# IlzeAmandaA/VAE-GP-ODE

Hardware: AMD Instinct MI355X
Metric: latent_trajectories_per_sec (higher is better)
Workload: dtype f32; 1 GPU; configs[1]: ode1 DF q=6 M=100 S=256 T=16 batch=256; step = full ELBO training step (encoder, GP draw, rk4 rollout, decoder, ELBO, backward, Adam), L=1; global_batch=256, mc_draws=1, solver=rk4 (3/8 rule), parallelism=dp1, hip_graph=True, graph_scope=whole, gp_side_stream=True, batchnorm=per-process statistics

## Files before the change

### include/gpode.h

```cpp
#ifndef GPODE_H
#define GPODE_H
#include <stddef.h>
#ifdef __cplusplus
extern "C" {
#endif

#define GPODE_KERNEL_RBF 0
#define GPODE_KERNEL_DF 1
#define GPODE_METHOD_EULER 0
#define GPODE_METHOD_RK4 1
#define GPODE_METHOD_MIDPOINT 2
#define GPODE_METHOD_DOPRI5 3

const char* gpode_version(void);
const char* gpode_last_error(void);
const char* gpode_last_launch(void);
int gpode_supported(int kernel, int Di, int Do);

int gpode_cache_sizes(int kernel, int Di, int Do, int M, int S, size_t* pack_floats, size_t* ws_floats);

int gpode_cache_build_fwd(int kernel, int Di, int Do, int M, int S,
                          const float* raw_ell, const float* raw_var, const float* Z,
                          const float* Um, const float* Us_packed,
                          const float* eps_u, const float* rff_w, const float* rff_eps, const float* rff_u,
// ... 170 lines not shown
                 int relu, float* scratch, void* stream);
int gpode_bn_stats(const float* x, const float* gamma, const float* beta, float* save_mean, float* save_invstd, float* running_mean,
                   float* running_var, long long* num_batches_tracked, float momentum, float eps, float* table, int B, int C, int HW,
                   float* scratch, void* stream);
int gpode_bn_moments(const float* x, float* moments, int B, int C, int HW, float* scratch, void* stream);
int gpode_bn_finalize(const float* gathered, int nranks, const float* gamma, const float* beta, float* save_mean, float* save_invstd,
                      float* running_mean, float* running_var, long long* num_batches_tracked, float momentum, float eps, float* table,
                      int C, void* stream);
int gpode_bn_apply(const float* x, const float* table, float* y, int B, int C, int HW, int relu, void* stream);
int gpode_bn_bwd_sums(const float* x, const float* gy, const float* gamma, const float* beta, const float* save_mean,
                      const float* save_invstd, float* sums, int B, int C, int HW, int relu, float* scratch, void* stream);
int gpode_bn_bwd_apply(const float* x, const float* gy, const float* gamma, const float* beta, const float* save_mean,
                       const float* save_invstd, const float* sums_gathered, const float* weights, int nranks, float count_all,
                       float* gx, float* ggamma, float* gbeta, float* gx_chansum, int B, int C, int HW, int relu, float* scratch,
                       void* stream);
void gpode_defer_reductions(int mode);
int gpode_flush_reductions(void* stream);
int gpode_dec10_bn_wgrad_scratch_floats(void);
int gpode_dec10_bn_bwd_sums_wgrad(const float* c, const float* gy, const float* w, const float* gamma, const float* beta, const float* save_mean,
                                  const float* save_invstd, float* sums, float* gw, float* gbias, int B, float* scratch, float* wscratch,
                                  void* stream);
int gpode_dec10_bn_scratch_floats(void);
int gpode_dec10_bn_bwd_sums(const float* c, const float* gy, const float* w, const float* gamma, const float* beta, const float* save_mean,
                            const float* save_invstd, float* sums, int B, float* scratch, void* stream);
int gpode_dec10_bn_bwd_apply(const float* c, const float* gy, const float* w, const float* gamma, const float* beta, const float* save_mean,
                             const float* save_invstd, const float* sums_gathered, const float* weights, int nranks, float count_all,
                             float* gc, float* ggamma, float* gbeta, float* gc_chansum, int B, float* scratch, void* stream);
int gpode_bn_eval(const float* x, const float* gy, const float* gamma, const float* beta, const float* running_mean,
                  const float* running_var, float eps, float* out, int B, int C, int HW, int relu, void* stream);
int gpode_bn_eval_table(const float* gamma, const float* beta, const float* running_mean, const float* running_var, float eps, float* table,
// ... 109 lines not shown
```

### vae-gp-ode_amd/_lib.py

```python
import ctypes
import os

_HERE = os.path.dirname(os.path.abspath(__file__))
LIB_PATH = os.path.join(_HERE, 'libgpode_hip.so')

_vp = ctypes.c_void_p
_i = ctypes.c_int
_f = ctypes.c_float
_sz = ctypes.c_size_t
_sz_p = ctypes.POINTER(_sz)

SIGNATURES = {
    'gpode_version': (ctypes.c_char_p, []),
    'gpode_last_error': (ctypes.c_char_p, []),
    'gpode_last_launch': (ctypes.c_char_p, []),
    'gpode_supported': (_i, [_i, _i, _i]),
    'gpode_cache_sizes': (_i, [_i, _i, _i, _i, _i, _sz_p, _sz_p]),
    'gpode_cache_build_fwd': (_i, [_i] * 5 + [_vp] * 20),
    'gpode_cache_bwd_sizes': (_i, [_i, _i, _i, _i, _i, _sz_p]),
    'gpode_cache_build_bwd': (_i, [_i] * 5 + [_vp] * 13 + [_i, _vp]),
    'gpode_cache_bwd_prepare': (_i, [_i] * 5 + [_vp] * 2 + [_vp]),
    'gpode_cache_info': (_i, [_vp, ctypes.POINTER(_i), _vp]),
    'gpode_cache_pivots': (_i, [_vp, ctypes.POINTER(_f), _vp]),
    'gpode_set_backward_solves': (_i, [_i]),
# ... 41 lines not shown
    'gpode_kern_cache': (_i, [_i] * 4 + [_vp] * 8 + [_vp]),
    'gpode_compute_nu_ws': (_i, [_i] * 4 + [_sz_p]),
    'gpode_compute_nu': (_i, [_i] * 4 + [_vp] * 5 + [_vp]),
    'gpode_f_update': (_i, [_i] * 4 + [_vp] * 5 + [_i, _vp, _vp, _vp]),
    'gpode_conv2d_fwd': (_i, [_vp] * 4 + [_i] * 10 + [_vp]),
    'gpode_conv2d_bwd_data': (_i, [_vp] * 4 + [_i] * 10 + [_vp]),
    'gpode_conv2d_fwd_bs': (_i, [_vp, _sz] + [_vp] * 3 + [_i] * 10 + [_vp]),
    'gpode_conv2d_bwd_weight_bs': (_i, [_vp, _sz] + [_vp] * 4 + [_i] * 10 + [_vp]),
    'gpode_convT_fwd_stats_scratch': (_sz, [_i]),
    'gpode_convT_fwd_stats': (_i, [_vp] * 5 + [_i] * 10 + [_vp] * 6 + [_vp, _f, _f, _vp, _vp, _i, _vp]),
    'gpode_conv_wgrad_scratch': (_sz, [_i, _i, _i, _i]),
    'gpode_conv2d_bwd_weight': (_i, [_vp] * 5 + [_i] * 10 + [_vp]),
    'gpode_bn_scratch': (_sz, [_i, _i]),
    'gpode_bn_fwd': (_i, [_vp] * 8 + [_vp, _f, _f, _i, _i, _i, _i, _vp, _vp]),
    'gpode_bn_bwd': (_i, [_vp] * 10 + [_i, _i, _i, _i, _vp, _vp]),
    'gpode_conv2d_bwd_data_bn': (_i, [_vp] * 5 + [_i] * 10 + [_vp]),
    'gpode_conv2d_bwd_weight_bn': (_i, [_vp] * 6 + [_i] * 10 + [_vp]),
    'gpode_bn_stats': (_i, [_vp] * 7 + [_vp, _f, _f, _vp, _i, _i, _i, _vp, _vp]),
    'gpode_bn_moments': (_i, [_vp, _vp, _i, _i, _i, _vp, _vp]),
    'gpode_bn_finalize': (_i, [_vp, _i] + [_vp] * 6 + [_vp, _f, _f, _vp, _i, _vp]),
    'gpode_bn_apply': (_i, [_vp, _vp, _vp, _i, _i, _i, _i, _vp]),
    'gpode_bn_bwd_sums': (_i, [_vp] * 7 + [_i, _i, _i, _i, _vp, _vp]),
    'gpode_bn_bwd_apply': (_i, [_vp] * 8 + [_i, _f] + [_vp] * 4 + [_i, _i, _i, _i, _vp, _vp]),
    'gpode_defer_reductions': (None, [_i]),
    'gpode_flush_reductions': (_i, [_vp]),
    'gpode_dec10_bn_scratch_floats': (_i, []),
    'gpode_dec10_bn_wgrad_scratch_floats': (_i, []),
    'gpode_dec10_bn_bwd_sums_wgrad': (_i, [_vp] * 10 + [_i, _vp, _vp, _vp]),
    'gpode_dec10_bn_bwd_sums': (_i, [_vp] * 8 + [_i, _vp, _vp]),
    'gpode_dec10_bn_bwd_apply': (_i, [_vp] * 9 + [_i, _f] + [_vp] * 4 + [_i, _vp, _vp]),
# ... 85 lines not shown
```

### vae-gp-ode_amd/csrc/capi.hip

```cpp
#include "../../include/gpode.h"
#include "gp_launch.hpp"

namespace gp {
char* error_slot() {
  static thread_local char buf[512] = {0};
  return buf;
}
const char** last_launch_slot() {
  static thread_local const char* tag = "";
  return &tag;
}
bool* force_substep_kernels() {
  static bool on = false;
  return &on;
}
}

extern "C" {

const char* gpode_version(void) { return "gpode-hip 0.1 (gfx950)"; }
const char* gpode_last_error(void) { return gp::error_slot(); }
const char* gpode_last_launch(void) { return *gp::last_launch_slot(); }
int gpode_supported(int kernel, int Di, int Do) { return gp::dims_supported(kernel, Di, Do); }

// ... 467 lines not shown
  if ((running_mean == nullptr) != (running_var == nullptr)) return gp::set_error("gpode_convT_fwd_stats: running_mean and running_var go together");
  return gp::convT_fwd_stats(x, x_bn, w, bias, y, GP_GEOM, gamma, beta, save_mean, save_invstd, running_mean, running_var, num_batches_tracked,
                             momentum, eps, table, scratch, slot, GP_ST);
}
size_t gpode_conv_wgrad_scratch(int B, int Ci, int Co, int K) { return gp::conv_wgrad_scratch(B, Ci, Co, K); }
int gpode_conv2d_bwd_weight(const float* x, const float* gy, float* gw, float* gbias, float* scratch, int B, int Ci, int H, int W,
                            int Co, int K, int S, int P, int Ho, int Wo, void* stream) {
  if (!x || !gy || !gw || !scratch) return gp::set_error("gpode_conv2d_bwd_weight: null pointer");
  return gp::conv2d_bwd_weight(x, gy, gw, gbias, scratch, GP_GEOM, nullptr, GP_ST);
}
int gpode_conv2d_bwd_weight_bn(const float* x, const float* gy, const float* gy_bn, float* gw, float* gbias, float* scratch, int B, int Ci,
                               int H, int W, int Co, int K, int S, int P, int Ho, int Wo, void* stream) {
  if (!x || !gy || !gy_bn || !gw || !scratch) return gp::set_error("gpode_conv2d_bwd_weight_bn: null pointer");
  return gp::conv2d_bwd_weight(x, gy, gw, gbias, scratch, GP_GEOM, gy_bn, GP_ST);
}
#undef GP_GEOM
size_t gpode_bn_scratch(int B, int C) { return gp::bn_scratch(B, C); }
int gpode_bn_fwd(const float* x, const float* gamma, const float* beta, float* y, float* save_mean, float* save_invstd,
                 float* running_mean, float* running_var, long long* num_batches_tracked, float momentum, float eps, int B, int C,
                 int HW, int relu, float* scratch, void* stream) {
  if (!x || !gamma || !beta || !y || !save_mean || !save_invstd || !scratch) return gp::set_error("gpode_bn_fwd: null pointer");
  return gp::bn_fwd(x, gamma, beta, y, save_mean, save_invstd, running_mean, running_var, num_batches_tracked, momentum, eps, B, C, HW, relu,
                    scratch, GP_ST);
}
int gpode_bn_bwd(const float* x, const float* gy, const float* gamma, const float* beta, const float* save_mean,
                 const float* save_invstd, float* gx, float* ggamma, float* gbeta, float* gx_chansum, int B, int C, int HW,
                 int relu, float* scratch, void* stream) {
  if (!x || !gy || !gamma || !beta || !save_mean || !save_invstd || !gx || !ggamma || !gbeta || !scratch)
    return gp::set_error("gpode_bn_bwd: null pointer");
  return gp::bn_bwd(x, gy, gamma, beta, save_mean, save_invstd, gx, ggamma, gbeta, gx_chansum, B, C, HW, relu, scratch, GP_ST);
}
int gpode_bn_stats(const float* x, const float* gamma, const float* beta, float* save_mean, float* save_invstd, float* running_mean,
                   float* running_var, long long* num_batches_tracked, float momentum, float eps, float* table, int B, int C, int HW,
                   float* scratch, void* stream) {
  if (!x || !gamma || !beta || !save_mean || !save_invstd || !table || !scratch) return gp::set_error("gpode_bn_stats: null pointer");
  return gp::bn_stats(x, gamma, beta, save_mean, save_invstd, running_mean, running_var, num_batches_tracked, momentum, eps, table, B, C, HW,
                      scratch, GP_ST);
}
int gpode_bn_moments(const float* x, float* moments, int B, int C, int HW, float* scratch, void* stream) {
  if (!x || !moments || !scratch) return gp::set_error("gpode_bn_moments: null pointer");
  return gp::bn_moments(x, moments, B, C, HW, scratch, GP_ST);
}
int gpode_bn_finalize(const float* gathered, int nranks, const float* gamma, const float* beta, float* save_mean, float* save_invstd,
                      float* running_mean, float* running_var, long long* num_batches_tracked, float momentum, float eps, float* table,
                      int C, void* stream) {
// ... 386 lines not shown
```

### vae-gp-ode_amd/csrc/conv_bwd_v2.hpp

```cpp
#pragma once
#include "conv_mfma.hpp"

namespace gp {

template <class L> struct BdV2 {
  using PL = BwdDataPolicy<L, L::CI>;
  static constexpr int KC = L::CO, NC = L::CI, KK = L::K * L::K;
  static constexpr int NCT = NC / 16;
  static constexpr int NKS = KK * (KC / 4);
  static constexpr int NPX = L::HI * L::HI;
  static constexpr int SRC = KC * L::HO * L::HO;
  static constexpr int PS = PL::PS, HP = PL::HP, IMG = KC * PS;
  static constexpr int CPS = NKS <= 100 ? 2 : 1;
  static constexpr int NCW = 4 * CPS, NTHR = 64 * (NCW + 4), NLT = NTHR - 64 * NCW;
  static constexpr int TSPLIT = NCW / NCT;
  static constexpr int TPW = CPS == 2 ? 2 : 4;
  static constexpr int WIN = 16 * TSPLIT * TPW;
  static constexpr int PF = 2;
  static constexpr int NTMIN = CPS == 2 ? 1 : TPW;
  static constexpr int NBUF = (2 * WIN - 2) / NPX + 2;
  static_assert(NCW % NCT == 0 && TSPLIT * NCT == NCW, "the consumers split the ci tiles evenly");
  static_assert(TPW * (PF + 1) <= 15, "LDS reads in flight within what lgkmcnt counts");
  static_assert(KC % 4 == 0 && SRC % 4 == 0, "float4 source");
  static constexpr bool ROW4 = L::HO % 4 == 0;
// ... 22 lines not shown
#pragma unroll
    for (int t = 0; t < NT; ++t) acc[t] = __builtin_amdgcn_mfma_f32_16x16x4f32(wr[s], bf[s % (E::PF + 1)][t], acc[t], 0, 0, 0);
    __builtin_amdgcn_sched_barrier(0);
  });
}

template <class E, int NT>
__device__ __forceinline__ void bdv2_window(int nt, const float* __restrict__ s_buf, const int (&base)[E::TPW], const float (&wr)[E::NKS],
                                            f32x4 (&acc)[E::TPW]) {
  if constexpr (NT > E::NTMIN) {
    if (nt < NT) { bdv2_window<E, NT - 1>(nt, s_buf, base, wr, acc); return; }
  }
  bdv2_tiles<E, NT>(s_buf, base, wr, acc);
}

template <class L>
__global__ __launch_bounds__(BdV2<L>::NTHR) void k_conv_bwd_data_v2(const float* __restrict__ gy, const float* __restrict__ w,
                                                                    float* __restrict__ gx, int B) {
  using E = BdV2<L>;
  using PL = typename E::PL;
  constexpr int KC = E::KC, NC = E::NC, KK = E::KK, NPX = E::NPX, IMG = E::IMG, PS = E::PS, HP = E::HP, WIN = E::WIN, NKS = E::NKS;
  constexpr int HO = L::HO, P = L::P, NLT = E::NLT, NBUF = E::NBUF, TPW = E::TPW, TSPLIT = E::TSPLIT;
  float* s_buf = igemm_smem;
  const int tid = threadIdx.x, lane = tid & 63, wave = __builtin_amdgcn_readfirstlane(tid >> 6);
  const int nit = ((int)blockIdx.x < B) ? (B - 1 - (int)blockIdx.x) / (int)gridDim.x + 1 : 0;
  const int npx = nit * NPX, nwin = (npx + WIN - 1) / WIN;
  auto last_img = [&](int i) { return min(nit - 1, (i * WIN + WIN - 1) / NPX); };

  for (int e = tid; e < NBUF * IMG / 4; e += E::NTHR) reinterpret_cast<float4*>(s_buf)[e] = float4{0.f, 0.f, 0.f, 0.f};
  __syncthreads();

  if (wave >= E::NCW) {
    __builtin_amdgcn_s_setprio(3);
// ... 28 lines not shown
        for (int g = 0; g < KC / 4; ++g) {
          float* d = buf + 4 * g * PS;
          d[otab[0]] = v[g].x; d[otab[1]] = v[g].y; d[otab[2]] = v[g].z; d[otab[3]] = v[g].w;
        }
      }
    };
    int staged = -1;
    if (nit > 0)
      for (; staged < last_img(0); ) stage(++staged);
    __syncthreads();
    for (int i = 0; i < nwin; ++i) {
      if (i + 1 < nwin)
        for (const int j1 = last_img(i + 1); staged < j1; ) stage(++staged);
      __syncthreads();
    }
    return;
  }

  const int lr = lane & 15, lk = lane >> 4, ct = wave / TSPLIT, sm = wave % TSPLIT;
  float wr[NKS];
#pragma unroll
  for (int s = 0; s < NKS; ++s) wr[s] = w[((size_t)(16 * ct + lr) * KC + 4 * (s % (KC / 4)) + lk) * KK + s / (KC / 4)];
  __syncthreads();
  for (int i = 0; i < nwin; ++i) {
    const int t0 = i * WIN + 16 * sm;
    int base[TPW], mm[TPW];
#pragma unroll
    for (int t = 0; t < TPW; ++t) {
      mm[t] = t0 + 16 * TSPLIT * t + lr;
      const int m = min(mm[t], npx - 1);
      const int j = m / NPX, p = m - j * NPX;
      base[t] = (j % NBUF) * IMG + lk * PS + PL::template C<0>::pix_addr(p);
    }
    f32x4 acc[TPW];
    const int nt = t0 < npx ? min(TPW, (npx - t0 + 16 * TSPLIT - 1) / (16 * TSPLIT)) : 0;
    if (nt > 0) bdv2_window<E, TPW>(nt, s_buf, base, wr, acc);
#pragma unroll
    for (int t = 0; t < TPW; ++t) {
      if (t < nt && mm[t] < npx) {
        const int j = mm[t] / NPX, p = mm[t] - j * NPX;
        float* o = gx + ((size_t)((int)blockIdx.x + j * (int)gridDim.x) * NC + 16 * ct + 4 * lk) * NPX + p;
#pragma unroll
        for (int r = 0; r < 4; ++r) o[(size_t)r * NPX] = acc[t][r];
      }
    }
    __syncthreads();
  }
}

}
```

### vae-gp-ode_amd/csrc/gp_launch.hpp

```cpp
#pragma once
#include <cstdint>
#include <cstdlib>
#include <hip/hip_runtime.h>
#include <cstdarg>
#include <cstdio>
#include <mutex>
#include <unordered_map>

namespace gp {

char* error_slot();
const char** last_launch_slot();

inline int set_error(const char* fmt, ...) {
  va_list ap;
  va_start(ap, fmt);
  vsnprintf(error_slot(), 512, fmt, ap);
  va_end(ap);
  return 1;
}

inline int check_launch(const char* what) {
  *last_launch_slot() = what;
  hipError_t e = hipGetLastError();
// ... 108 lines not shown
                   const float* Us_packed, const float* x, int cov_mode, float* mean, float* var, float* ws, hipStream_t st);
int svgp_kl_fwd(int M, int Do, const float* Um, const float* Us, float* kl, hipStream_t st);
int noise_fill(float* out, long long n_normal, long long n_uniform, unsigned long long seed, unsigned long long* state, hipStream_t st);
int svgp_kl_bwd(int M, int Do, const float* Um, const float* Us, const float* g, float* dUm, float* dUs, hipStream_t st);

void set_backward_solves(int mode);
int get_backward_solves();
int cache_bwd_sizes(int kernel, int Di, int Do, int M, int S, int nd, size_t* bws_floats);
int cache_build_bwd(int kernel, int Di, int Do, int M, int S, int nd, const float* raw_ell, const float* raw_var, const float* Z,
                    const float* eps_u, const float* pack, const float* ws, float* gpack, float* bws,
                    float* g_raw_ell, float* g_raw_var, float* g_Z, float* g_Um, float* g_Us, int prepared, hipStream_t st);
int cache_bwd_prepare(int kernel, int Di, int Do, int M, int S, int nd, const float* ws, float* bws, hipStream_t st);

struct ConvGeom { int B, Ci, H, W, Co, K, S, P, Ho, Wo; };
int conv2d_fwd(const float* x, const float* w, const float* bias, float* y, const ConvGeom& g, hipStream_t st, size_t xbs = 0);
size_t convT_fwd_stats_scratch(int Co_out);
int convT_fwd_stats(const float* x, const float* x_bn, const float* w, const float* bias, float* y, const ConvGeom& g, const float* gamma,
                    const float* beta, float* save_mean, float* save_invstd, float* running_mean, float* running_var, long long* nbt,
                    float momentum, float eps, float* table, float* scratch, int slot, hipStream_t st);
int conv2d_bwd_data(const float* gy, const float* w, const float* bias, float* gx, const ConvGeom& g, const float* gy_bn, hipStream_t st);
size_t conv_wgrad_scratch(int B, int Ci, int Co, int K);
int conv2d_bwd_weight(const float* x, const float* gy, float* gw, float* gbias, float* scratch, const ConvGeom& g, const float* gy_bn,
                      hipStream_t st, size_t xbs = 0);
size_t bn_scratch(int B, int C);
int bn_fwd(const float* x, const float* gamma, const float* beta, float* y, float* save_mean, float* save_invstd,
           float* running_mean, float* running_var, long long* num_batches_tracked, float momentum, float eps, int B, int C, int HW,
           int relu, float* scratch, hipStream_t st);
int bn_bwd(const float* x, const float* gy, const float* gamma, const float* beta, const float* save_mean, const float* save_invstd,
           float* gx, float* ggamma, float* gbeta, float* gx_chansum, int B, int C, int HW, int relu, float* scratch, hipStream_t st);
int bn_stats(const float* x, const float* gamma, const float* beta, float* save_mean, float* save_invstd, float* running_mean,
             float* running_var, long long* num_batches_tracked, float momentum, float eps, float* table, int B, int C, int HW,
             float* scratch, hipStream_t st);
int bn_moments(const float* x, float* mom, int B, int C, int HW, float* scratch, hipStream_t st);
int bn_finalize(const float* gathered, int W, const float* gamma, const float* beta, float* save_mean, float* save_invstd,
                float* running_mean, float* running_var, long long* num_batches_tracked, float momentum, float eps, float* table, int C,
                hipStream_t st);
int bn_apply(const float* x, const float* table, float* y, int B, int C, int HW, int relu, hipStream_t st);
int dec10_bn_scratch_floats();
int dec10_bn_bwd_sums(const float* c, const float* gy, const float* w, const float* gamma, const float* beta, const float* mean,
                      const float* invstd, float* sums, int B, float* scratch, hipStream_t st, float* gw = nullptr, float* wscratch = nullptr, float* gbias = nullptr);
int dec10_bn_wgrad_scratch_floats();
int dec10_bn_bwd_apply(const float* c, const float* gy, const float* w, const float* gamma, const float* beta, const float* mean,
                       const float* invstd, const float* gathered, const float* wts, int W, float count_all, float* gc, float* ggamma,
                       float* gbeta, float* gc_chansum, int B, float* scratch, hipStream_t st);
// ... 87 lines not shown
```

### vae-gp-ode_amd/csrc/vae_conv_tiled.hip

```cpp
#include <hip/hip_runtime.h>
#include <cstdlib>
#include "gp_launch.hpp"
#include "conv_layers.hpp"
#include "conv_mfma.hpp"
#include "conv_dec10_mfma.hpp"
#include "conv_dec1_mfma.hpp"
#include "conv_dec4_mfma.hpp"

namespace gp {

extern __shared__ __attribute__((aligned(16))) float tsm[];

template <class L, int IPB>
__global__ __launch_bounds__(256) void k_convT_fwd(const float* __restrict__ x, const float* __restrict__ w,
                                                    const float* __restrict__ bias, float* __restrict__ y, int B) {
  constexpr int CI = L::CI, CO = L::CO, HI = L::HI, HO = L::HO, HP = L::HP, K = L::K, S = L::S, P = L::P, PL = L::PL;
  constexpr int CPT = CO % 16 == 0 ? 16 : 8;
  static_assert(CO % CPT == 0, "8 or 16 output channels per thread");
  constexpr int NG = CO / CPT;
  constexpr int IMG = CI * HP * HP;
  float* s_img = tsm;
  float* s_w = tsm + IPB * IMG;
  const int tid = threadIdx.x;
  const int b0 = blockIdx.x * IPB;
// ... 443 lines not shown
      else hipLaunchKernelGGL(dec10::k_fwd<false>, B < num_cus() ? B : num_cus(), 512, ldsm, st, gy, w, bias, gx, B, in_bn);
      return check_launch("dec10_fwd_mfma");
    }
    if (in_bn) return set_error("convT forward with a fused BatchNorm input needs the matrix-core path (16-byte aligned operands, GPODE_CONV_VALU unset)");
    if (!aligned16(gx)) return -1;
    constexpr int IPB = 2;
    const size_t lds = sizeof(float) * ((size_t)IPB * 16 * 32 * 32 + 16 * 5 * 8);
    auto kern = k_dec10_fwd<IPB>;
    if (set_max_lds((const void*)kern, lds)) return 1;
    hipLaunchKernelGGL(kern, (B + IPB - 1) / IPB, 256, lds, st, gy, w, bias, gx, B);
    return check_launch("dec10_fwd");
  }
  return -1;
}

int tiled_fwd(const float* x, const float* w, const float* bias, float* y, const ConvGeom& g, hipStream_t st) {
  if (g.H != g.W || g.Ho != g.Wo) return -1;
  const int B = g.B;
  const bool mfma = use_mfma() && aligned16(x, w, y);
  if (mfma) {
    if (matches<Enc3>(g)) return launch_igemm<BwdDataPolicy<Enc3, 16>, 4, 4, 1>(x, w, bias, y, B, st, "enc_conv3_fwd_mfma");
    if (matches<Enc6>(g)) return launch_igemm<BwdDataPolicy<Enc6, 32>, 8, 1, 2>(x, w, bias, y, B, st, "enc_conv6_fwd_mfma");
  }
  if (bias) return -1;
  if (matches<Dec7>(g)) {
    if (mfma && !conv_v1()) return conv_v2_dec7_bwd_data(x, w, y, B, st);
    if (mfma) return launch_igemm<BwdDataPolicy<Dec7, 16>, 1, 2, 1, false, 256>(x, w, nullptr, y, B, st, "convT_bwd_data_mfma");
    return launch_T2<Dec7, 2, 8>(x, w, y, B, st);
  }
  if (matches<Dec4>(g)) {
// ... 190 lines not shown
```

### vae-gp-ode_amd/csrc/vae_conv_v2.hip

```cpp
#include <hip/hip_runtime.h>
#include <cstdint>
#include "gp_launch.hpp"
#include "conv_layers.hpp"
#include "conv_bwd_v2.hpp"
#include "conv_fwd_v2.hpp"

namespace gp {

template <class L> static int launch_bwd_data_v2(const float* gy, const float* w, float* gx, int B, hipStream_t st, const char* what) {
  using E = BdV2<L>;
  constexpr size_t lds = E::lds_bytes();
  static_assert(lds <= 160 * 1024, "LDS budget");
  auto km = k_conv_bwd_data_v2<L>;
  if (set_max_lds((const void*)km, lds)) return 1;
  hipLaunchKernelGGL(km, B < num_cus() ? B : num_cus(), E::NTHR, lds, st, gy, w, gx, B);
  return check_launch(what);
}

int conv_v2_dec7_bwd_data(const float* gy, const float* w, float* gx, int B, hipStream_t st) {
  return launch_bwd_data_v2<Dec7>(gy, w, gx, B, st, "conv_v2_dec7_bwd_data");
}

int conv_v2_dec4_bwd_data(const float* gy, const float* w, float* gx, int B, hipStream_t st) {
  return launch_bwd_data_v2<Dec4>(gy, w, gx, B, st, "conv_v2_dec4_bwd_data");
}

template <class L, bool HAS_BN, bool STATS>
static int launch_fwd_v2(const float* x, const float* w, const float* bias, float* y, int B, const float* in_bn, const BnSink* sink,
                         hipStream_t st, const char* what) {
  using E = FwV2<L>;
  constexpr size_t lds = E::lds_bytes(STATS);
  static_assert(lds + (STATS ? sizeof(float) * (E::NTHR + 1) : 0) <= 160 * 1024, "LDS budget (with bn_sink_publish's static arrays)");
  auto km = k_conv_fwd_v2<L, HAS_BN, STATS>;
  if (set_max_lds((const void*)km, lds)) return 1;
  if (STATS && num_cus() > 512) return set_error("%s: more workgroups than the statistics scratch holds", what);
// ... 15 lines not shown
```

### vae-gp-ode_amd/csrc/vae_norm.hip

```cpp
#include <hip/hip_runtime.h>
#include <mutex>
#include "gp_launch.hpp"
#include "wave_reduce.hpp"
#include "bn_math.hpp"

namespace gp {

namespace {

template <class F4, class F1>
__device__ __forceinline__ void chan_slab(int C, int HW, int c, int b0, int nb, F4&& f4, F1&& f1) {
  if ((HW & 3) == 0) {
    const int hw4 = HW >> 2, work = nb * hw4;
    int q = threadIdx.x, b = q / hw4, p = q - b * hw4;
    const int sb = 256 / hw4, sp = 256 - sb * hw4;
#pragma unroll 4
    for (; q < work; q += 256) {
      f4(((size_t)(b0 + b) * C + c) * HW + 4 * p);
      p += sp; b += sb;
      if (p >= hw4) { p -= hw4; ++b; }
    }
  } else {
    const int work = nb * HW;
    int q = threadIdx.x, b = q / HW, p = q - b * HW;
// ... 9 lines not shown

template <int NV> __device__ __forceinline__ void block_sum_store(const float (&v)[NV], float* __restrict__ dst) {
  __shared__ float red[4][NV];
  float out[NV];
  wave_sum_multi<NV>(v, out);
  if ((threadIdx.x & 63) == 0) {
#pragma unroll
    for (int i = 0; i < NV; ++i) red[threadIdx.x >> 6][i] = out[i];
  }
  __syncthreads();
  if (threadIdx.x < NV) dst[threadIdx.x] = (red[0][threadIdx.x] + red[1][threadIdx.x]) + (red[2][threadIdx.x] + red[3][threadIdx.x]);
}

__device__ __forceinline__ void split_sums(const float* __restrict__ part, int nsplit, int C, int c, float& a, float& b) {
  const int lane = threadIdx.x & 63;
  const float in2[2] = {lane < nsplit ? part[((size_t)lane * C + c) * 2] : 0.f, lane < nsplit ? part[((size_t)lane * C + c) * 2 + 1] : 0.f};
  float out2[2];
  wave_sum_multi<2>(in2, out2);
  a = out2[0];
  b = out2[1];
}

__device__ __forceinline__ float chan_shift(const float* __restrict__ x, int HW, int c) {
  const int n = HW < 64 ? HW : 64, lane = threadIdx.x & 63;
  const float in1[1] = {lane < n ? x[(size_t)c * HW + lane] : 0.f};
  float out1[1];
  wave_sum_multi<1>(in1, out1);
  return out1[0] / (float)n;
}

__global__ __launch_bounds__(256) void k_bn_stats(const float* __restrict__ x, int B, int C, int HW, int bps, float* __restrict__ part,
// ... 427 lines not shown
  if ((HW & 3) == 0 && !(aligned16(x) && aligned16(gy) && aligned16(gx))) return set_error("gpode_bn_bwd: x / gy / gx must be 16-byte aligned");
  if (bn_small((size_t)B * HW, kBnSmallBwd)) {
    hipLaunchKernelGGL(k_bn_bwd_small, C, 256, 0, st, x, gy, gamma, beta, save_mean, save_invstd, (float)B * HW, ggamma, gbeta, gx, gx_chansum, B, C,
                       HW, relu);
    return check_launch("bn_bwd (one launch)");
  }
  const Split sp = pick(B);
  hipLaunchKernelGGL(k_bn_bwd_sums, dim3(C, sp.used), 256, 0, st, x, gy, gamma, beta, save_mean, save_invstd, B, C, HW, sp.bps, relu, scratch);
  float* part_gx = gx_chansum ? scratch + (size_t)sp.ns * C * 2 + (size_t)C * 3 : nullptr;
  hipLaunchKernelGGL(k_bn_bwd_apply, dim3(C, sp.used), 256, 0, st, x, gy, gamma, beta, save_mean, save_invstd, scratch, sp.used, (float)B * HW,
                     ggamma, gbeta, gx, part_gx, B, C, HW, sp.bps, relu, (const float*)nullptr, (const float*)nullptr, 0);
  if (gx_chansum && reduce_job(RedJob{part_gx, gx_chansum, sp.used, C, 2, 0, 0, 0}, st)) return 1;
  return check_launch("bn_bwd");
}

int bn_moments(const float* x, float* mom, int B, int C, int HW, float* scratch, hipStream_t st) {
  if ((HW & 3) == 0 && !aligned16(x)) return set_error("gpode_bn_moments: x must be 16-byte aligned");
  const Split sp = pick(B);
  float* shift = scratch + (size_t)sp.ns * C * 2 + (size_t)C * 2;
  hipLaunchKernelGGL(k_bn_stats, dim3(C, sp.used), 256, 0, st, x, B, C, HW, sp.bps, scratch, shift);
  hipLaunchKernelGGL(k_bn_moments, C + 1, 64, 0, st, scratch, shift, sp.used, C, (float)B * HW, mom);
  return check_launch("bn_moments");
}

int bn_finalize(const float* gathered, int W, const float* gamma, const float* beta, float* save_mean, float* save_invstd,
                float* running_mean, float* running_var, long long* num_batches_tracked, float momentum, float eps, float* table, int C,
                hipStream_t st) {
  if (W < 1 || W > 64) return set_error("gpode_bn_finalize: %d ranks (1..64 supported)", W);
  hipLaunchKernelGGL(k_bn_finalize, C, 64, 0, st, gathered, W, gamma, beta, C, eps, momentum, save_mean, save_invstd, running_mean, running_var,
                     num_batches_tracked, table);
// ... 157 lines not shown
```

### vae-gp-ode_amd/vae_ops.py

```python
import ctypes
import os

import torch

from . import _lib, ops
from .ops import _chk, _ptr, _stream




def _new(shape, like):
    return torch.empty(shape, dtype=torch.float32, device=like.device)


def _bchw(x):
    return x.shape[0], x.shape[1], x[0, 0].numel()


def _convT_out(Hi, Wi, K, stride, pad, out_pad):
    return (Hi - 1) * stride - 2 * pad + K + out_pad, (Wi - 1) * stride - 2 * pad + K + out_pad


def _scratch(n, like):
    return torch.empty(max(int(n), 4), dtype=torch.float32, device=like.device)
# ... 109 lines not shown

def _bn_global_bwd(sync, x, gy, gamma, beta, mean, invstd, relu):
    sums, gy, scratch = _bn_bwd_sums(x, gy, gamma, beta, mean, invstd, relu)
    return _bn_bwd_apply(sync, sync.gather(sums), scratch, x, gy, gamma, beta, mean, invstd, relu)


def _bn_bwd(sync, x, gy, gamma, beta, mean, invstd, relu):
    if sync is not None:
        return _bn_global_bwd(sync, x, gy, gamma, beta, mean, invstd, relu)
    B, C, HW = _bchw(x)
    gx, gg, gb, cs = _new(x.shape, x), _new((C,), x), _new((C,), x), _new((C,), x)
    bs = _bn_scratch(B, C, x)
    _bwd_call('gpode_bn_bwd', _ptr(x), _ptr(gy.contiguous()), _ptr(gamma), _ptr(beta), _ptr(mean), _ptr(invstd), _ptr(gx), _ptr(gg),
              _ptr(gb), _ptr(cs), B, C, HW, relu, _ptr(bs), _stream(), keep=(bs,))
    return gx, gg, gb, cs


_pack_bn = {'on': os.environ.get('GPODE_PACK_BN_GATHERS', '0') == '1'}


def set_pack_bn_gathers(on):
    _pack_bn['on'] = bool(on)


def pack_bn_gathers():
    return _pack_bn['on'] and _bn_sync is not None


class _BatchNormTrainPair(torch.autograd.Function):

# ... 233 lines not shown
            if not gw_rides:
                ws = _wgrad_scratch(B, Cout, Cin, K, c)
                _bwd_call('gpode_conv2d_bwd_weight_bn', _ptr(gy), _ptr(c), _ptr(table), _ptr(gw), _ptr(None),
                          _ptr(ws), B, Cout, Ht, Wt, Cin, K, S, P, Hi, Wi, _stream(), keep=(ws,))
            gb = _fused_chansum(gy, Cout) if has_b else None
        to_sum = has_b and gw is not None and gb is None
        if to_sum:
            gb = _new((Cout,), c)
            if not gw_rides:
                bs = _bn_scratch(B, Cout, c)
                _bwd_call('gpode_chan_sum', _ptr(gy), _ptr(gb), B, Cout, Ht * Wt, _ptr(bs), _stream(), keep=(bs,))
        gb_rides = gb if (to_sum and gw_rides) else None
        if last_stage:
            gc, gg, gbeta, cs = _dec10_bn_bwd(ctx.sync, c, gy, w, gamma, beta, mean, invstd, gw=gw if gw_rides else None, gbias=gb_rides)
        else:
            ga = _new(c.shape, c)
            _lib.call('gpode_conv2d_fwd', _ptr(gy), _ptr(w), _ptr(None), _ptr(ga), B, Cout, Ht, Wt, Cin, K, S, P, Hi, Wi, _stream())
            gc, gg, gbeta, cs = _bn_bwd(ctx.sync, c, ga, gamma, beta, mean, invstd, 1)
        gc._gpode_chansum = cs
        return gc, gg, gbeta, None, None, None, None, None, gw, gb, None, None, None, None, None


class _BatchNormTrain(torch.autograd.Function):
    @staticmethod
    def forward(ctx, x, gamma, beta, running_mean, running_var, momentum, eps, relu, nbt=None):
        x = _chk(x, 'x')
        B, C, HW = _bchw(x)
        if nbt is not None and not (nbt.is_cuda and nbt.dtype == torch.int64):
            raise _lib.GpodeError('num_batches_tracked must be an int64 CUDA/HIP scalar')
        ctx.sync = _bn_sync
        if _bn_sync is not None:
            mean, invstd, table = _bn_global_stats(x, gamma, beta, running_mean, running_var, nbt, momentum, eps)
            y = _bn_apply(x, table, relu)
# ... 779 lines not shown
```

Measured before the change: 110,100 trajectories/s.

## Fuse BN backward channel sums into the dec7 conv data-gradient epilogue

The dec7 convolution backward-data kernel now also computes the per-block ReLU-masked batchnorm backward partial sums (sum of g and sum of g*xhat) in its epilogue. A new bn_bwd_from_parts entry point applies the BN backward using those partials, so the separate reduction pass over the data gradient is skipped. The fused path is used only when running without a BN sync and when the operands are 16-byte aligned. The cost is extra loads of x inside the conv kernel, extra registers and one LDS reduction, and split_sums is extended to handle more than 64 partial rows.

Measured after the change: 111,200 trajectories/s (median of 6 runs). Within noise of the previous version (+1.0%).

```diff
diff --git a/include/gpode.h b/include/gpode.h
--- a/include/gpode.h
+++ b/include/gpode.h
@@ -208,6 +208,13 @@
                        const float* save_invstd, const float* sums_gathered, const float* weights, int nranks, float count_all,
                        float* gx, float* ggamma, float* gbeta, float* gx_chansum, int B, int C, int HW, int relu, float* scratch,
                        void* stream);
+size_t gpode_conv2d_fwd_bnsums_scratch(int B, int Ci, int H, int W, int Co, int K, int S, int P, int Ho, int Wo);
+int gpode_conv2d_fwd_bnsums(const float* x, const float* w, const float* bias, float* y, int B, int Ci, int H, int W, int Co,
+                            int K, int S, int P, int Ho, int Wo, const float* x_bn, const float* table, float* part, int* nsplit_out,
+                            void* stream);
+int gpode_bn_bwd_from_parts(const float* x, const float* gy, const float* gamma, const float* beta, const float* save_mean,
+                            const float* save_invstd, const float* part, int nsplit, float* gx, float* ggamma, float* gbeta,
+                            float* gx_chansum, int B, int C, int HW, int relu, float* scratch, void* stream);
 void gpode_defer_reductions(int mode);
 int gpode_flush_reductions(void* stream);
 int gpode_dec10_bn_wgrad_scratch_floats(void);
diff --git a/vae-gp-ode_amd/_lib.py b/vae-gp-ode_amd/_lib.py
--- a/vae-gp-ode_amd/_lib.py
+++ b/vae-gp-ode_amd/_lib.py
@@ -79,6 +79,9 @@
     'gpode_bn_scratch': (_sz, [_i, _i]),
     'gpode_bn_fwd': (_i, [_vp] * 8 + [_vp, _f, _f, _i, _i, _i, _i, _vp, _vp]),
     'gpode_bn_bwd': (_i, [_vp] * 10 + [_i, _i, _i, _i, _vp, _vp]),
+    'gpode_conv2d_fwd_bnsums_scratch': (_sz, [_i] * 10),
+    'gpode_conv2d_fwd_bnsums': (_i, [_vp] * 4 + [_i] * 10 + [_vp] * 3 + [ctypes.POINTER(_i), _vp]),
+    'gpode_bn_bwd_from_parts': (_i, [_vp] * 7 + [_i] + [_vp] * 4 + [_i, _i, _i, _i, _vp, _vp]),
     'gpode_conv2d_bwd_data_bn': (_i, [_vp] * 5 + [_i] * 10 + [_vp]),
     'gpode_conv2d_bwd_weight_bn': (_i, [_vp] * 6 + [_i] * 10 + [_vp]),
     'gpode_bn_stats': (_i, [_vp] * 7 + [_vp, _f, _f, _vp, _i, _i, _i, _vp, _vp]),
diff --git a/vae-gp-ode_amd/csrc/capi.hip b/vae-gp-ode_amd/csrc/capi.hip
--- a/vae-gp-ode_amd/csrc/capi.hip
+++ b/vae-gp-ode_amd/csrc/capi.hip
@@ -505,6 +505,16 @@
   if (!x || !gy || !gy_bn || !gw || !scratch) return gp::set_error("gpode_conv2d_bwd_weight_bn: null pointer");
   return gp::conv2d_bwd_weight(x, gy, gw, gbias, scratch, GP_GEOM, gy_bn, GP_ST);
 }
+size_t gpode_conv2d_fwd_bnsums_scratch(int B, int Ci, int H, int W, int Co, int K, int S, int P, int Ho, int Wo) {
+  return (size_t)gp::conv2d_fwd_bnsums_splits(GP_GEOM) * Co * 2;
+}
+int gpode_conv2d_fwd_bnsums(const float* x, const float* w, const float* bias, float* y, int B, int Ci, int H, int W, int Co,
+                            int K, int S, int P, int Ho, int Wo, const float* x_bn, const float* table, float* part, int* nsplit_out,
+                            void* stream) {
+  if (!x || !w || !y || !x_bn || !table || !part || !nsplit_out) return gp::set_error("gpode_conv2d_fwd_bnsums: null pointer");
+  if (bias) return gp::set_error("gpode_conv2d_fwd_bnsums: no specialisation with a bias");
+  return gp::conv2d_fwd_bnsums(x, w, y, GP_GEOM, x_bn, table, part, nsplit_out, GP_ST);
+}
 #undef GP_GEOM
 size_t gpode_bn_scratch(int B, int C) { return gp::bn_scratch(B, C); }
 int gpode_bn_fwd(const float* x, const float* gamma, const float* beta, float* y, float* save_mean, float* save_invstd,
@@ -520,6 +530,14 @@
   if (!x || !gy || !gamma || !beta || !save_mean || !save_invstd || !gx || !ggamma || !gbeta || !scratch)
     return gp::set_error("gpode_bn_bwd: null pointer");
   return gp::bn_bwd(x, gy, gamma, beta, save_mean, save_invstd, gx, ggamma, gbeta, gx_chansum, B, C, HW, relu, scratch, GP_ST);
+}
+int gpode_bn_bwd_from_parts(const float* x, const float* gy, const float* gamma, const float* beta, const float* save_mean,
+                            const float* save_invstd, const float* part, int nsplit, float* gx, float* ggamma, float* gbeta,
+                            float* gx_chansum, int B, int C, int HW, int relu, float* scratch, void* stream) {
+  if (!x || !gy || !gamma || !beta || !save_mean || !save_invstd || !part || !gx || !ggamma || !gbeta || !scratch)
+    return gp::set_error("gpode_bn_bwd_from_parts: null pointer");
+  return gp::bn_bwd_from_parts(x, gy, gamma, beta, save_mean, save_invstd, part, nsplit, gx, ggamma, gbeta, gx_chansum, B, C, HW, relu, scratch,
+                               GP_ST);
 }
 int gpode_bn_stats(const float* x, const float* gamma, const float* beta, float* save_mean, float* save_invstd, float* running_mean,
                    float* running_var, long long* num_batches_tracked, float momentum, float eps, float* table, int B, int C, int HW,
diff --git a/vae-gp-ode_amd/csrc/conv_bwd_v2.hpp b/vae-gp-ode_amd/csrc/conv_bwd_v2.hpp
--- a/vae-gp-ode_amd/csrc/conv_bwd_v2.hpp
+++ b/vae-gp-ode_amd/csrc/conv_bwd_v2.hpp
@@ -1,5 +1,7 @@
 #pragma once
 #include "conv_mfma.hpp"
+#include "bn_math.hpp"
+#include "wave_reduce.hpp"
 
 namespace gp {
 
@@ -60,9 +62,12 @@
   bdv2_tiles<E, NT>(s_buf, base, wr, acc);
 }
 
-template <class L>
+template <bool BNSUMS> struct BnSumsArgs {};
+template <> struct BnSumsArgs<true> { const float* x; const float* table; float* part; };
+
+template <class L, bool BNSUMS = false>
 __global__ __launch_bounds__(BdV2<L>::NTHR) void k_conv_bwd_data_v2(const float* __restrict__ gy, const float* __restrict__ w,
-                                                                    float* __restrict__ gx, int B) {
+                                                                    float* __restrict__ gx, int B, BnSumsArgs<BNSUMS> bn) {
   using E = BdV2<L>;
   using PL = typename E::PL;
   constexpr int KC = E::KC, NC = E::NC, KK = E::KK, NPX = E::NPX, IMG = E::IMG, PS = E::PS, HP = E::HP, WIN = E::WIN, NKS = E::NKS;
@@ -121,6 +126,7 @@
         for (const int j1 = last_img(i + 1); staged < j1; ) stage(++staged);
       __syncthreads();
     }
+    if constexpr (BNSUMS) __syncthreads();
     return;
   }
 
@@ -128,16 +134,28 @@
   float wr[NKS];
 #pragma unroll
   for (int s = 0; s < NKS; ++s) wr[s] = w[((size_t)(16 * ct + lr) * KC + 4 * (s % (KC / 4)) + lk) * KK + s / (KC / 4)];
+  float4 tb[4];
+  float s0[4] = {0.f, 0.f, 0.f, 0.f}, s1[4] = {0.f, 0.f, 0.f, 0.f};
+  if constexpr (BNSUMS) {
+#pragma unroll
+    for (int r = 0; r < 4; ++r) tb[r] = reinterpret_cast<const float4*>(bn.table)[16 * ct + 4 * lk + r];
+  }
   __syncthreads();
   for (int i = 0; i < nwin; ++i) {
     const int t0 = i * WIN + 16 * sm;
     int base[TPW], mm[TPW];
+    float xv[TPW][4];
 #pragma unroll
     for (int t = 0; t < TPW; ++t) {
       mm[t] = t0 + 16 * TSPLIT * t + lr;
       const int m = min(mm[t], npx - 1);
       const int j = m / NPX, p = m - j * NPX;
       base[t] = (j % NBUF) * IMG + lk * PS + PL::template C<0>::pix_addr(p);
+      if constexpr (BNSUMS) {
+        const float* xi = bn.x + ((size_t)((int)blockIdx.x + j * (int)gridDim.x) * NC + 16 * ct + 4 * lk) * NPX + p;
+#pragma unroll
+        for (int r = 0; r < 4; ++r) xv[t][r] = xi[(size_t)r * NPX];
+      }
     }
     f32x4 acc[TPW];
     const int nt = t0 < npx ? min(TPW, (npx - t0 + 16 * TSPLIT - 1) / (16 * TSPLIT)) : 0;
@@ -149,10 +167,35 @@
         float* o = gx + ((size_t)((int)blockIdx.x + j * (int)gridDim.x) * NC + 16 * ct + 4 * lk) * NPX + p;
 #pragma unroll
         for (int r = 0; r < 4; ++r) o[(size_t)r * NPX] = acc[t][r];
+        if constexpr (BNSUMS) {
+#pragma unroll
+          for (int r = 0; r < 4; ++r) {
+            const float xh = bn_xhat(xv[t][r], tb[r].x, tb[r].y);
+            const float g = (__fmaf_rn(xh, tb[r].z, tb[r].w) > 0.f) ? acc[t][r] : 0.f;
+            s0[r] += g;
+            s1[r] = fmaf(g, xh, s1[r]);
+          }
+        }
       }
     }
     __syncthreads();
   }
-}
-
-}
+  if constexpr (BNSUMS) {
+    float* red = s_buf;
+#pragma unroll
+    for (int r = 0; r < 4; ++r) {
+      const float a = row_allreduce16(s0[r]), b = row_allreduce16(s1[r]);
+      if (lr == 0) { red[((wave * 4 + lk) * 4 + r) * 2] = a; red[((wave * 4 + lk) * 4 + r) * 2 + 1] = b; }
+    }
+    __syncthreads();
+    if (tid < 2 * NC) {
+      const int c = tid >> 1, h = tid & 1, q = c & 15;
+      float v = red[((((c >> 4) * TSPLIT) * 4 + (q >> 2)) * 4 + (q & 3)) * 2 + h];
+#pragma unroll
+      for (int sm2 = 1; sm2 < TSPLIT; ++sm2) v += red[((((c >> 4) * TSPLIT + sm2) * 4 + (q >> 2)) * 4 + (q & 3)) * 2 + h];
+      bn.part[((size_t)blockIdx.x * NC + c) * 2 + h] = v;
+    }
+  }
+}
+
+}
diff --git a/vae-gp-ode_amd/csrc/gp_launch.hpp b/vae-gp-ode_amd/csrc/gp_launch.hpp
--- a/vae-gp-ode_amd/csrc/gp_launch.hpp
+++ b/vae-gp-ode_amd/csrc/gp_launch.hpp
@@ -146,6 +146,9 @@
 
 struct ConvGeom { int B, Ci, H, W, Co, K, S, P, Ho, Wo; };
 int conv2d_fwd(const float* x, const float* w, const float* bias, float* y, const ConvGeom& g, hipStream_t st, size_t xbs = 0);
+int conv2d_fwd_bnsums_splits(const ConvGeom& g);
+int conv2d_fwd_bnsums(const float* x, const float* w, float* y, const ConvGeom& g, const float* x_bn, const float* table, float* part,
+                      int* nsplit_out, hipStream_t st);
 size_t convT_fwd_stats_scratch(int Co_out);
 int convT_fwd_stats(const float* x, const float* x_bn, const float* w, const float* bias, float* y, const ConvGeom& g, const float* gamma,
                     const float* beta, float* save_mean, float* save_invstd, float* running_mean, float* running_var, long long* nbt,
@@ -160,6 +163,9 @@
            int relu, float* scratch, hipStream_t st);
 int bn_bwd(const float* x, const float* gy, const float* gamma, const float* beta, const float* save_mean, const float* save_invstd,
            float* gx, float* ggamma, float* gbeta, float* gx_chansum, int B, int C, int HW, int relu, float* scratch, hipStream_t st);
+int bn_bwd_from_parts(const float* x, const float* gy, const float* gamma, const float* beta, const float* save_mean,
+                      const float* save_invstd, const float* part, int nsplit, float* gx, float* ggamma, float* gbeta, float* gx_chansum,
+                      int B, int C, int HW, int relu, float* scratch, hipStream_t st);
 int bn_stats(const float* x, const float* gamma, const float* beta, float* save_mean, float* save_invstd, float* running_mean,
              float* running_var, long long* num_batches_tracked, float momentum, float eps, float* table, int B, int C, int HW,
              float* scratch, hipStream_t st);
diff --git a/vae-gp-ode_amd/csrc/vae_conv_tiled.hip b/vae-gp-ode_amd/csrc/vae_conv_tiled.hip
--- a/vae-gp-ode_amd/csrc/vae_conv_tiled.hip
+++ b/vae-gp-ode_amd/csrc/vae_conv_tiled.hip
@@ -481,6 +481,23 @@
   return -1;
 }
 
+int conv_v2_dec7_bwd_data_bnsums(const float* gy, const float* w, float* gx, int B, const float* x, const float* table, float* part,
+                                 hipStream_t st);
+int conv2d_fwd_bnsums_splits(const ConvGeom& g) {
+  if (g.B < 1 || g.H != g.W || g.Ho != g.Wo || !matches<Dec7>(g) || !use_mfma() || conv_v1()) return 0;
+  const int nwg = g.B < num_cus() ? g.B : num_cus();
+  return nwg <= 256 ? nwg : 0;
+}
+int conv2d_fwd_bnsums(const float* x, const float* w, float* y, const ConvGeom& g, const float* x_bn, const float* table, float* part,
+                      int* nsplit_out, hipStream_t st) {
+  const int nwg = conv2d_fwd_bnsums_splits(g);
+  if (!nwg) return set_error("gpode_conv2d_fwd_bnsums: no specialisation for this geometry (or the second convolution engine is switched off)");
+  if (!aligned16(x, w, y, table)) return set_error("gpode_conv2d_fwd_bnsums: no specialisation for operands (x, w, y, table) that are not 16-byte aligned");
+  if (conv_v2_dec7_bwd_data_bnsums(x, w, y, g.B, x_bn, table, part, st)) return 1;
+  *nsplit_out = nwg;
+  return 0;
+}
+
 int tiled_fwd(const float* x, const float* w, const float* bias, float* y, const ConvGeom& g, hipStream_t st) {
   if (g.H != g.W || g.Ho != g.Wo) return -1;
   const int B = g.B;
diff --git a/vae-gp-ode_amd/csrc/vae_conv_v2.hip b/vae-gp-ode_amd/csrc/vae_conv_v2.hip
--- a/vae-gp-ode_amd/csrc/vae_conv_v2.hip
+++ b/vae-gp-ode_amd/csrc/vae_conv_v2.hip
@@ -13,12 +13,29 @@
   static_assert(lds <= 160 * 1024, "LDS budget");
   auto km = k_conv_bwd_data_v2<L>;
   if (set_max_lds((const void*)km, lds)) return 1;
-  hipLaunchKernelGGL(km, B < num_cus() ? B : num_cus(), E::NTHR, lds, st, gy, w, gx, B);
+  hipLaunchKernelGGL(km, B < num_cus() ? B : num_cus(), E::NTHR, lds, st, gy, w, gx, B, BnSumsArgs<false>{});
+  return check_launch(what);
+}
+
+template <class L> static int launch_bwd_data_v2_bnsums(const float* gy, const float* w, float* gx, int B, const float* x, const float* table,
+                                                        float* part, hipStream_t st, const char* what) {
+  using E = BdV2<L>;
+  constexpr size_t lds = E::lds_bytes();
+  static_assert(lds <= 160 * 1024 && sizeof(float) * E::NCW * 32 <= lds, "LDS budget; the consumers' sums fit the plane buffers");
+  static_assert(2 * L::CI <= 64 * E::NCW, "the final sums are written by consumer threads");
+  auto km = k_conv_bwd_data_v2<L, true>;
+  if (set_max_lds((const void*)km, lds)) return 1;
+  hipLaunchKernelGGL(km, B < num_cus() ? B : num_cus(), E::NTHR, lds, st, gy, w, gx, B, BnSumsArgs<true>{x, table, part});
   return check_launch(what);
 }
 
 int conv_v2_dec7_bwd_data(const float* gy, const float* w, float* gx, int B, hipStream_t st) {
   return launch_bwd_data_v2<Dec7>(gy, w, gx, B, st, "conv_v2_dec7_bwd_data");
+}
+
+int conv_v2_dec7_bwd_data_bnsums(const float* gy, const float* w, float* gx, int B, const float* x, const float* table, float* part,
+                                 hipStream_t st) {
+  return launch_bwd_data_v2_bnsums<Dec7>(gy, w, gx, B, x, table, part, st, "conv_v2_dec7_bwd_data_bnsums");
 }
 
 int conv_v2_dec4_bwd_data(const float* gy, const float* w, float* gx, int B, hipStream_t st) {
diff --git a/vae-gp-ode_amd/csrc/vae_norm.hip b/vae-gp-ode_amd/csrc/vae_norm.hip
--- a/vae-gp-ode_amd/csrc/vae_norm.hip
+++ b/vae-gp-ode_amd/csrc/vae_norm.hip
@@ -47,7 +47,11 @@
 
 __device__ __forceinline__ void split_sums(const float* __restrict__ part, int nsplit, int C, int c, float& a, float& b) {
   const int lane = threadIdx.x & 63;
-  const float in2[2] = {lane < nsplit ? part[((size_t)lane * C + c) * 2] : 0.f, lane < nsplit ? part[((size_t)lane * C + c) * 2 + 1] : 0.f};
+  float in2[2] = {lane < nsplit ? part[((size_t)lane * C + c) * 2] : 0.f, lane < nsplit ? part[((size_t)lane * C + c) * 2 + 1] : 0.f};
+  for (int s = lane + 64; s < nsplit; s += 64) {
+    in2[0] += part[((size_t)s * C + c) * 2];
+    in2[1] += part[((size_t)s * C + c) * 2 + 1];
+  }
   float out2[2];
   wave_sum_multi<2>(in2, out2);
   a = out2[0];
@@ -505,6 +509,20 @@
   return check_launch("bn_bwd");
 }
 
+int bn_bwd_from_parts(const float* x, const float* gy, const float* gamma, const float* beta, const float* save_mean,
+                      const float* save_invstd, const float* part, int nsplit, float* gx, float* ggamma, float* gbeta, float* gx_chansum,
+                      int B, int C, int HW, int relu, float* scratch, hipStream_t st) {
+  if (nsplit < 1 || nsplit > 256) return set_error("gpode_bn_bwd_from_parts: %d rows of partial sums (1..256 supported)", nsplit);
+  if (B < 1 || C < 1 || HW < 1) return set_error("gpode_bn_bwd_from_parts: B, C, HW >= 1");
+  if ((HW & 3) == 0 && !(aligned16(x) && aligned16(gy) && aligned16(gx))) return set_error("gpode_bn_bwd_from_parts: x / gy / gx must be 16-byte aligned");
+  const Split sp = bn_small((size_t)B * HW, kBnSmallBwd) ? Split{1, B, 1} : pick(B);
+  float* part_gx = gx_chansum ? scratch + (size_t)sp.ns * C * 2 + (size_t)C * 3 : nullptr;
+  hipLaunchKernelGGL(k_bn_bwd_apply, dim3(C, sp.used), 256, 0, st, x, gy, gamma, beta, save_mean, save_invstd, part, nsplit, (float)B * HW,
+                     ggamma, gbeta, gx, part_gx, B, C, HW, sp.bps, relu, (const float*)nullptr, (const float*)nullptr, 0);
+  if (gx_chansum && reduce_job(RedJob{part_gx, gx_chansum, sp.used, C, 2, 0, 0, 0}, st)) return 1;
+  return check_launch("bn_bwd_from_parts");
+}
+
 int bn_moments(const float* x, float* mom, int B, int C, int HW, float* scratch, hipStream_t st) {
   if ((HW & 3) == 0 && !aligned16(x)) return set_error("gpode_bn_moments: x must be 16-byte aligned");
   const Split sp = pick(B);
diff --git a/vae-gp-ode_amd/vae_ops.py b/vae-gp-ode_amd/vae_ops.py
--- a/vae-gp-ode_amd/vae_ops.py
+++ b/vae-gp-ode_amd/vae_ops.py
@@ -147,6 +147,24 @@
     _bwd_call('gpode_bn_bwd', _ptr(x), _ptr(gy.contiguous()), _ptr(gamma), _ptr(beta), _ptr(mean), _ptr(invstd), _ptr(gx), _ptr(gg),
               _ptr(gb), _ptr(cs), B, C, HW, relu, _ptr(bs), _stream(), keep=(bs,))
     return gx, gg, gb, cs
+
+
+def _conv_bwd_bnsums_floats(geom, *operands):
+    if any(t.data_ptr() % 16 for t in operands):
+        return 0
+    return _lib.load().gpode_conv2d_fwd_bnsums_scratch(*geom)
+
+
+def _conv_bn_bwd(c, gy, w, gamma, beta, mean, invstd, table, geom, nfloats):
+    B, C, HW = _bchw(c)
+    ga, part, nsplit = _new(c.shape, c), _scratch(nfloats, c), ctypes.c_int(0)
+    _lib.call('gpode_conv2d_fwd_bnsums', _ptr(gy), _ptr(w), _ptr(None), _ptr(ga), *geom, _ptr(c), _ptr(table), _ptr(part),
+              ctypes.byref(nsplit), _stream())
+    gc, gg, gb, cs = _new(c.shape, c), _new((C,), c), _new((C,), c), _new((C,), c)
+    bs = _bn_scratch(B, C, c)
+    _bwd_call('gpode_bn_bwd_from_parts', _ptr(c), _ptr(ga), _ptr(gamma), _ptr(beta), _ptr(mean), _ptr(invstd), _ptr(part), nsplit.value,
+              _ptr(gc), _ptr(gg), _ptr(gb), _ptr(cs), B, C, HW, 1, _ptr(bs), _stream(), keep=(bs, part))
+    return gc, gg, gb, cs
 
 
 _pack_bn = {'on': os.environ.get('GPODE_PACK_BN_GATHERS', '0') == '1'}
@@ -410,9 +428,14 @@
         if last_stage:
             gc, gg, gbeta, cs = _dec10_bn_bwd(ctx.sync, c, gy, w, gamma, beta, mean, invstd, gw=gw if gw_rides else None, gbias=gb_rides)
         else:
-            ga = _new(c.shape, c)
-            _lib.call('gpode_conv2d_fwd', _ptr(gy), _ptr(w), _ptr(None), _ptr(ga), B, Cout, Ht, Wt, Cin, K, S, P, Hi, Wi, _stream())
-            gc, gg, gbeta, cs = _bn_bwd(ctx.sync, c, ga, gamma, beta, mean, invstd, 1)
+            geom = (B, Cout, Ht, Wt, Cin, K, S, P, Hi, Wi)
+            nfloats = _conv_bwd_bnsums_floats(geom, gy, w, c, table) if ctx.sync is None else 0
+            if nfloats:
+                gc, gg, gbeta, cs = _conv_bn_bwd(c, gy, w, gamma, beta, mean, invstd, table, geom, nfloats)
+            else:
+                ga = _new(c.shape, c)
+                _lib.call('gpode_conv2d_fwd', _ptr(gy), _ptr(w), _ptr(None), _ptr(ga), *geom, _stream())
+                gc, gg, gbeta, cs = _bn_bwd(ctx.sync, c, ga, gamma, beta, mean, invstd, 1)
         gc._gpode_chansum = cs
         return gc, gg, gbeta, None, None, None, None, None, gw, gb, None, None, None, None, None
 
```
